# ZrrSkywalker/MonoDETR

Measured on NVIDIA H100. Metric: images/sec (1280x384, fwd+bwd), higher is better.
Workload: dtype f32 (BF16x3: error-compensated bf16 tensor-core products, fp32 accumulate)

## Files before the change

monodetr_b200/csrc/attention.cu:

```cuda
#include <cuda_runtime.h>
#include <math.h>
#include <stdint.h>

#include "../../include/monodetr_b200.h"
#include "launch.cuh"
#include "rng.cuh"
#include "tc_common.cuh"

namespace {

using namespace mdb;

constexpr int HD = 32;
constexpr int BR = 64;
constexpr int BC = 64;
constexpr int kTileBytes = BC * HD * 4;
constexpr int ATT_THREADS = 128;

struct AttnParams {
    const float *q, *k, *v;
    const uint8_t* kpm;
    float* out;
    float* lse;
    int B, H, Lq, Lk, ldq, ldk, ldv, ldo;
    float scale;
    float drop_p;
    const unsigned long long* seed;
    unsigned long long site;
    const float *dout, *o;
    float* delta;
    float *dq, *dk, *dv;
    int lddq, lddk, lddv;
};

__device__ __forceinline__ uint32_t f2tf32(float x) {
    uint32_t r;
    asm("cvt.rna.tf32.f32 %0, %1;" : "=r"(r) : "f"(x));
    return r;
}
__device__ __forceinline__ void split_tf32(float x, uint32_t& hi, uint32_t& lo) {
    hi = f2tf32(x);
    lo = f2tf32(x - __uint_as_float(hi));
}
struct AFrag {
    uint32_t hi[4][4];
    uint32_t lo[4][4];
};
__device__ __forceinline__ void load_afrag(AFrag& f, const float* base, int ld, int r0, int nrows, int lane, float mul) {
    const int g = lane >> 2, t = lane & 3;
    const int ra = r0 + g, rb = r0 + g + 8;
    const float* pa = base + (size_t)min(ra, nrows - 1) * ld;
    const float* pb = base + (size_t)min(rb, nrows - 1) * ld;
    const float ma = ra < nrows ? mul : 0.f, mb = rb < nrows ? mul : 0.f;
#pragma unroll
    for (int ks = 0; ks < 4; ++ks) {
        split_tf32(pa[ks * 8 + t] * ma, f.hi[ks][0], f.lo[ks][0]);
        split_tf32(pb[ks * 8 + t] * mb, f.hi[ks][1], f.lo[ks][1]);
        split_tf32(pa[ks * 8 + t + 4] * ma, f.hi[ks][2], f.lo[ks][2]);
        split_tf32(pb[ks * 8 + t + 4] * mb, f.hi[ks][3], f.lo[ks][3]);
    }
}

__device__ __forceinline__ uint32_t nt_off(int r, int c) { return (uint32_t)(r * 128 + ((((c >> 2) ^ (r & 7))) << 4) + (c & 3) * 4); }
__device__ __forceinline__ uint32_t nn_off(int r, int c) {
    const int kk = r & 31, q = kk & 7;
    const int kpos = (kk & ~7) + ((q & 1) ? 4 + (q >> 1) : (q >> 1));
    return (uint32_t)((r >> 5) * 4096 + c * 128 + ((((kpos >> 2) ^ (c & 7))) << 4) + (kpos & 3) * 4);
}

template <int NS>
__device__ __forceinline__ void gemm_nt(float (&c)[8][4], const AFrag& a, uint32_t th, uint32_t tl) {
    float (&d)[32] = reinterpret_cast<float (&)[32]>(c);
#pragma unroll
    for (int i = 0; i < 32; ++i) d[i] = 0.f;
    wgmma_fence();
#pragma unroll
    for (int ks = 0; ks < 4; ++ks) {
        const uint64_t bh = make_wgmma_desc_sw128(th + ks * 32);
        if (NS == 3) {
            const uint64_t bl = make_wgmma_desc_sw128(tl + ks * 32);
            wgmma_tf32_n64(d, a.lo[ks], bh, 1);
            wgmma_tf32_n64(d, a.hi[ks], bl, 1);
        }
        wgmma_tf32_n64(d, a.hi[ks], bh, 1);
    }
    wgmma_commit();
    wgmma_wait_all();
    wgmma_fence_operands(d);
}

template <int NS>
__device__ __forceinline__ void gemm_nn(float (&acc)[4][4], const float (&p)[8][4], uint32_t th, uint32_t tl) {
    float (&d)[16] = reinterpret_cast<float (&)[16]>(acc);
#pragma unroll
    for (int half = 0; half < 2; ++half) {
        uint32_t ah[4][4], al[4][4];
#pragma unroll
        for (int u = 0; u < 4; ++u) {
            const int kt = half * 4 + u;
            split_tf32(p[kt][0], ah[u][0], al[u][0]);
            split_tf32(p[kt][2], ah[u][1], al[u][1]);
            split_tf32(p[kt][1], ah[u][2], al[u][2]);
            split_tf32(p[kt][3], ah[u][3], al[u][3]);
        }
        wgmma_fence();
#pragma unroll
        for (int u = 0; u < 4; ++u) {
            const uint32_t off = half * 4096 + u * 32;
            const uint64_t bh = make_wgmma_desc_sw128(th + off);
            if (NS == 3) {
                const uint64_t bl = make_wgmma_desc_sw128(tl + off);
                wgmma_tf32_n32(d, al[u], bh, 1);
                wgmma_tf32_n32(d, ah[u], bl, 1);
            }
            wgmma_tf32_n32(d, ah[u], bh, 1);
        }
        wgmma_commit();
        wgmma_wait_all();
        wgmma_fence_operands(d);
    }
}

constexpr int STG = BC * HD;
__device__ __forceinline__ void stage_tile(float* stg, const float* base, int ld, int r0, int nrows) {
#pragma unroll
    for (int u = 0; u < 4; ++u) {
        const int i = threadIdx.x + u * ATT_THREADS;
        const int r = i >> 3, c = (i & 7) * 4;
        const bool ok = r0 + r < nrows;
        const float* src = ok ? base + ((size_t)(r0 + r) * ld + c) : base;
        const uint32_t dst = (uint32_t)__cvta_generic_to_shared(stg) + (uint32_t)i * 16u;
        const int nbytes = ok ? 16 : 0;
        asm volatile("cp.async.cg.shared.global [%0], [%1], 16, %2;" ::"r"(dst), "l"(src), "r"(nbytes) : "memory");
    }
}
__device__ __forceinline__ void stage_commit() { asm volatile("cp.async.commit_group;" ::: "memory"); }
__device__ __forceinline__ void stage_wait() { asm volatile("cp.async.wait_all;" ::: "memory"); }
__device__ __forceinline__ void unstage_tile(uint8_t* nt_hi, uint8_t* nt_lo, uint8_t* nn_hi, uint8_t* nn_lo, const float* stg) {
#pragma unroll
    for (int u = 0; u < 4; ++u) {
        const int i = threadIdx.x + u * ATT_THREADS;
        const int r = i >> 3, c = (i & 7) * 4;
        const float4 v = *reinterpret_cast<const float4*>(stg + i * 4);
        uint32_t h[4], l[4];
        split_tf32(v.x, h[0], l[0]); split_tf32(v.y, h[1], l[1]); split_tf32(v.z, h[2], l[2]); split_tf32(v.w, h[3], l[3]);
        if (nt_hi) *reinterpret_cast<uint4*>(nt_hi + nt_off(r, c)) = make_uint4(h[0], h[1], h[2], h[3]);
        if (nt_lo) *reinterpret_cast<uint4*>(nt_lo + nt_off(r, c)) = make_uint4(l[0], l[1], l[2], l[3]);
#pragma unroll
        for (int e = 0; e < 4; ++e) {
            if (nn_hi) *reinterpret_cast<uint32_t*>(nn_hi + nn_off(r, c + e)) = h[e];
            if (nn_lo) *reinterpret_cast<uint32_t*>(nn_lo + nn_off(r, c + e)) = l[e];
        }
    }
}
static_assert(BC * (HD / 4) == 4 * ATT_THREADS, "tile loader mapping");

__device__ __forceinline__ float quad_max(float v) {
    v = fmaxf(v, __shfl_xor_sync(0xffffffffu, v, 1));
    return fmaxf(v, __shfl_xor_sync(0xffffffffu, v, 2));
}
__device__ __forceinline__ float quad_sum(float v) {
    v += __shfl_xor_sync(0xffffffffu, v, 1);
    return v + __shfl_xor_sync(0xffffffffu, v, 2);
}

struct DropCtx {
    uint32_t key, thr;
    float inv_keep;
    bool on;
};
__device__ __forceinline__ DropCtx make_drop(const AttnParams& p, int b, int h) {
    DropCtx d;
    d.on = p.drop_p > 0.f;
    d.inv_keep = 1.f / (1.f - p.drop_p);
    d.thr = mdb::rng_thr16(p.drop_p);
    d.key = 0u;
    if (d.on) d.key = mdb::rng_key32(*p.seed + p.site * 0x9E3779B97F4A7C15ull, (unsigned long long)(b * p.H + h));
    return d;
}
__device__ __forceinline__ float keep_scale(const DropCtx& d, uint32_t row_base, int j) {
    return mdb::rng_keep16(d.key, row_base + (uint32_t)j, d.thr) ? d.inv_keep : 0.f;
}

__device__ __forceinline__ uint32_t fetch_dead(const AttnParams& p, int b, int k0) {
    const int j = k0 + (int)threadIdx.x;
    if (threadIdx.x >= BC) return 0u;
    if (j >= p.Lk) return 1u;
    return (p.kpm && p.kpm[(size_t)b * p.Lk + j]) ? 1u : 0u;
}

__global__ void __launch_bounds__(ATT_THREADS, 3)
attn_fwd_kernel(const AttnParams p) {
    extern __shared__ __align__(1024) uint8_t dyn_smem[];
    uint8_t* sKh = dyn_smem;
    uint8_t* sKl = sKh + kTileBytes;
    uint8_t* sVh = sKl + kTileBytes;
    uint8_t* sVl = sVh + kTileBytes;
    float* gK = reinterpret_cast<float*>(sVl + kTileBytes);
    float* gV = gK + STG;
    uint8_t* sDead = reinterpret_cast<uint8_t*>(gV + STG);
    const int b = blockIdx.z, h = blockIdx.y;
    const int warp = threadIdx.x >> 5, lane = threadIdx.x & 31;
    const int g = lane >> 2, t = lane & 3;
    const int r0 = blockIdx.x * BR + warp * 16;
    const float* qb = p.q + (size_t)b * p.Lq * p.ldq + h * HD;
    const float* kb = p.k + (size_t)b * p.Lk * p.ldk + h * HD;
    const float* vb = p.v + (size_t)b * p.Lk * p.ldv + h * HD;
    const DropCtx drop = make_drop(p, b, h);
    stage_tile(gK, kb, p.ldk, 0, p.Lk);
    stage_tile(gV, vb, p.ldv, 0, p.Lk);
    stage_commit();
    uint32_t ndead = fetch_dead(p, b, 0);
    AFrag qa;
    load_afrag(qa, qb, p.ldq, r0, p.Lq, lane, p.scale);
    float acc[4][4];
#pragma unroll
    for (int i = 0; i < 4; ++i) acc[i][0] = acc[i][1] = acc[i][2] = acc[i][3] = 0.f;
    float m0 = -INFINITY, m1 = -INFINITY, l0 = 0.f, l1 = 0.f;
    const int qi0 = r0 + g, qi1 = r0 + g + 8;
    const uint32_t rb0 = (uint32_t)qi0 * (uint32_t)p.Lk, rb1 = (uint32_t)qi1 * (uint32_t)p.Lk;

    for (int k0 = 0; k0 < p.Lk; k0 += BC) {
        stage_wait();
        __syncthreads();
        unstage_tile(sKh, sKl, nullptr, nullptr, gK);
        unstage_tile(nullptr, nullptr, sVh, sVl, gV);
        if (threadIdx.x < BC) sDead[threadIdx.x] = (uint8_t)ndead;
        mdb::fence_proxy_async_smem();
        __syncthreads();
        if (k0 + BC < p.Lk) {
            stage_tile(gK, kb, p.ldk, k0 + BC, p.Lk);
            stage_tile(gV, vb, p.ldv, k0 + BC, p.Lk);
            stage_commit();
            ndead = fetch_dead(p, b, k0 + BC);
        }
        float s[8][4];
        gemm_nt<3>(s, qa, mdb::smem_u32(sKh), mdb::smem_u32(sKl));
        float mx0 = -INFINITY, mx1 = -INFINITY;
#pragma unroll
        for (int nt = 0; nt < 8; ++nt) {
            const uchar2 dd = *reinterpret_cast<const uchar2*>(&sDead[nt * 8 + 2 * t]);
            if (dd.x) { s[nt][0] = -INFINITY; s[nt][2] = -INFINITY; }
            if (dd.y) { s[nt][1] = -INFINITY; s[nt][3] = -INFINITY; }
            mx0 = fmaxf(mx0, fmaxf(s[nt][0], s[nt][1]));
            mx1 = fmaxf(mx1, fmaxf(s[nt][2], s[nt][3]));
        }
        const float mn0 = fmaxf(m0, quad_max(mx0)), mn1 = fmaxf(m1, quad_max(mx1));
        const float c0 = (mn0 == -INFINITY) ? 1.f : __expf(m0 - mn0), c1 = (mn1 == -INFINITY) ? 1.f : __expf(m1 - mn1);
        l0 *= c0; l1 *= c1;
#pragma unroll
        for (int dn = 0; dn < 4; ++dn) { acc[dn][0] *= c0; acc[dn][1] *= c0; acc[dn][2] *= c1; acc[dn][3] *= c1; }
#pragma unroll
        for (int nt = 0; nt < 8; ++nt) {
#pragma unroll
            for (int e = 0; e < 2; ++e) {
                const int j = k0 + nt * 8 + 2 * t + e;
                float p0 = (mn0 == -INFINITY) ? 0.f : __expf(s[nt][e] - mn0);
                float p1 = (mn1 == -INFINITY) ? 0.f : __expf(s[nt][2 + e] - mn1);
                l0 += p0; l1 += p1;
                if (drop.on) {
                    p0 *= keep_scale(drop, rb0, j);
                    p1 *= keep_scale(drop, rb1, j);
                }
                s[nt][e] = p0; s[nt][2 + e] = p1;
            }
        }
        m0 = mn0; m1 = mn1;
        gemm_nn<3>(acc, s, mdb::smem_u32(sVh), mdb::smem_u32(sVl));
    }
    l0 = quad_sum(l0); l1 = quad_sum(l1);
    const float i0 = l0 > 0.f ? 1.f / l0 : 0.f, i1 = l1 > 0.f ? 1.f / l1 : 0.f;
    float* ob = p.out + (size_t)b * p.Lq * p.ldo + h * HD;
#pragma unroll
    for (int dn = 0; dn < 4; ++dn) {
        if (qi0 < p.Lq) *reinterpret_cast<float2*>(ob + (size_t)qi0 * p.ldo + dn * 8 + 2 * t) = make_float2(acc[dn][0] * i0, acc[dn][1] * i0);
        if (qi1 < p.Lq) *reinterpret_cast<float2*>(ob + (size_t)qi1 * p.ldo + dn * 8 + 2 * t) = make_float2(acc[dn][2] * i1, acc[dn][3] * i1);
    }
    if (t == 0) {
        float* lp = p.lse + ((size_t)b * p.H + h) * p.Lq;
        if (qi0 < p.Lq) lp[qi0] = l0 > 0.f ? m0 + __logf(l0) : -INFINITY;
        if (qi1 < p.Lq) lp[qi1] = l1 > 0.f ? m1 + __logf(l1) : -INFINITY;
    }
}

__global__ void attn_delta_kernel(const AttnParams p) {
    const long long idx = blockIdx.x * (long long)blockDim.x + threadIdx.x;
    const long long n = (long long)p.B * p.Lq * p.H;
    if (idx >= n) return;
    const int h = (int)(idx % p.H);
    const long long bi = idx / p.H;
    const int i = (int)(bi % p.Lq);
    const int b = (int)(bi / p.Lq);
    const float* a = p.dout + (size_t)bi * p.ldo + h * HD;
    const float* o = p.o + (size_t)bi * p.ldo + h * HD;
    float s = 0.f;
#pragma unroll
    for (int d = 0; d < HD; d += 4) {
        const float4 x = *reinterpret_cast<const float4*>(a + d);
        const float4 y = *reinterpret_cast<const float4*>(o + d);
        s += x.x * y.x + x.y * y.y + x.z * y.z + x.w * y.w;
    }
    p.delta[((size_t)b * p.H + h) * p.Lq + i] = s;
}

__global__ void __launch_bounds__(ATT_THREADS, 3)
attn_bwd_dq_kernel(const AttnParams p) {
    extern __shared__ __align__(1024) uint8_t dyn_smem[];
    uint8_t* sKh = dyn_smem;
    uint8_t* sKl = sKh + kTileBytes;
    uint8_t* sKn = sKl + kTileBytes;
    uint8_t* sVh = sKn + kTileBytes;
    float* gK = reinterpret_cast<float*>(sVh + kTileBytes);
    float* gV = gK + STG;
    uint8_t* sDead = reinterpret_cast<uint8_t*>(gV + STG);
    const int b = blockIdx.z, h = blockIdx.y;
    const int warp = threadIdx.x >> 5, lane = threadIdx.x & 31;
    const int g = lane >> 2, t = lane & 3;
    const int r0 = blockIdx.x * BR + warp * 16;
    const float* qb = p.q + (size_t)b * p.Lq * p.ldq + h * HD;
    const float* gb = p.dout + (size_t)b * p.Lq * p.ldo + h * HD;
    const float* kb = p.k + (size_t)b * p.Lk * p.ldk + h * HD;
    const float* vb = p.v + (size_t)b * p.Lk * p.ldv + h * HD;
    const DropCtx drop = make_drop(p, b, h);
    stage_tile(gK, kb, p.ldk, 0, p.Lk);
    stage_tile(gV, vb, p.ldv, 0, p.Lk);
    stage_commit();
    uint32_t ndead = fetch_dead(p, b, 0);
    AFrag qa, ga;
    load_afrag(qa, qb, p.ldq, r0, p.Lq, lane, p.scale);
    load_afrag(ga, gb, p.ldo, r0, p.Lq, lane, 1.f);
    const int qi0 = r0 + g, qi1 = r0 + g + 8;
    const uint32_t rb0 = (uint32_t)qi0 * (uint32_t)p.Lk, rb1 = (uint32_t)qi1 * (uint32_t)p.Lk;
    const size_t st = ((size_t)b * p.H + h) * p.Lq;
    float lse0 = qi0 < p.Lq ? p.lse[st + qi0] : INFINITY, lse1 = qi1 < p.Lq ? p.lse[st + qi1] : INFINITY;
    if (lse0 == -INFINITY) lse0 = INFINITY;
    if (lse1 == -INFINITY) lse1 = INFINITY;
    const float dl0 = qi0 < p.Lq ? p.delta[st + qi0] : 0.f, dl1 = qi1 < p.Lq ? p.delta[st + qi1] : 0.f;
    float acc[4][4];
#pragma unroll
    for (int i = 0; i < 4; ++i) acc[i][0] = acc[i][1] = acc[i][2] = acc[i][3] = 0.f;

    for (int k0 = 0; k0 < p.Lk; k0 += BC) {
        stage_wait();
        __syncthreads();
        unstage_tile(sKh, sKl, sKn, nullptr, gK);
        unstage_tile(sVh, nullptr, nullptr, nullptr, gV);
        if (threadIdx.x < BC) sDead[threadIdx.x] = (uint8_t)ndead;
        mdb::fence_proxy_async_smem();
        __syncthreads();
        if (k0 + BC < p.Lk) {
            stage_tile(gK, kb, p.ldk, k0 + BC, p.Lk);
            stage_tile(gV, vb, p.ldv, k0 + BC, p.Lk);
            stage_commit();
            ndead = fetch_dead(p, b, k0 + BC);
        }
        float s[8][4], dp[8][4];
        gemm_nt<3>(s, qa, mdb::smem_u32(sKh), mdb::smem_u32(sKl));
        gemm_nt<1>(dp, ga, mdb::smem_u32(sVh), 0u);
#pragma unroll
        for (int nt = 0; nt < 8; ++nt) {
            const uchar2 dd = *reinterpret_cast<const uchar2*>(&sDead[nt * 8 + 2 * t]);
#pragma unroll
            for (int e = 0; e < 2; ++e) {
                const int j = k0 + nt * 8 + 2 * t + e;
                const bool dead = e ? dd.y : dd.x;
                float p0 = dead ? 0.f : __expf(s[nt][e] - lse0);
                float p1 = dead ? 0.f : __expf(s[nt][2 + e] - lse1);
                float d0 = dp[nt][e], d1 = dp[nt][2 + e];
                if (drop.on) {
                    d0 *= keep_scale(drop, rb0, j);
                    d1 *= keep_scale(drop, rb1, j);
                }
                s[nt][e] = p0 * (d0 - dl0);
                s[nt][2 + e] = p1 * (d1 - dl1);
            }
        }
        gemm_nn<1>(acc, s, mdb::smem_u32(sKn), 0u);
    }
    float* ob = p.dq + (size_t)b * p.Lq * p.lddq + h * HD;
#pragma unroll
    for (int dn = 0; dn < 4; ++dn) {
        if (qi0 < p.Lq) *reinterpret_cast<float2*>(ob + (size_t)qi0 * p.lddq + dn * 8 + 2 * t) = make_float2(acc[dn][0] * p.scale, acc[dn][1] * p.scale);
        if (qi1 < p.Lq) *reinterpret_cast<float2*>(ob + (size_t)qi1 * p.lddq + dn * 8 + 2 * t) = make_float2(acc[dn][2] * p.scale, acc[dn][3] * p.scale);
    }
}

__global__ void __launch_bounds__(ATT_THREADS, 2)
attn_bwd_dkv_kernel(const AttnParams p) {
    extern __shared__ __align__(1024) uint8_t dyn_smem[];
    uint8_t* sQh = dyn_smem;
    uint8_t* sQl = sQh + kTileBytes;
    uint8_t* sQn = sQl + kTileBytes;
    uint8_t* sGh = sQn + kTileBytes;
    uint8_t* sGn = sGh + kTileBytes;
    float* gQ = reinterpret_cast<float*>(sGn + kTileBytes);
    float* gG = gQ + STG;
    float* sL = gG + STG;
    float* sD = sL + BC;
    const int b = blockIdx.z, h = blockIdx.y;
    const int warp = threadIdx.x >> 5, lane = threadIdx.x & 31;
    const int g = lane >> 2, t = lane & 3;
    const int r0 = blockIdx.x * BR + warp * 16;
    const float* qb = p.q + (size_t)b * p.Lq * p.ldq + h * HD;
    const float* gb = p.dout + (size_t)b * p.Lq * p.ldo + h * HD;
    const float* kb = p.k + (size_t)b * p.Lk * p.ldk + h * HD;
    const float* vb = p.v + (size_t)b * p.Lk * p.ldv + h * HD;
    const DropCtx drop = make_drop(p, b, h);
    const size_t st = ((size_t)b * p.H + h) * p.Lq;
    auto fetch_stats = [&](int q0, float& l, float& d) {
        const int i = q0 + (int)threadIdx.x;
        l = INFINITY; d = 0.f;
        if (threadIdx.x < BC && i < p.Lq) {
            l = p.lse[st + i];
            d = p.delta[st + i];
            if (l == -INFINITY) l = INFINITY;
        }
    };
    float nl, nd;
    stage_tile(gQ, qb, p.ldq, 0, p.Lq);
    stage_tile(gG, gb, p.ldo, 0, p.Lq);
    stage_commit();
    fetch_stats(0, nl, nd);
    AFrag ka, va;
    load_afrag(ka, kb, p.ldk, r0, p.Lk, lane, p.scale);
    load_afrag(va, vb, p.ldv, r0, p.Lk, lane, 1.f);
    const int kj0 = r0 + g, kj1 = r0 + g + 8;
    const bool dead0 = kj0 >= p.Lk || (p.kpm && p.kpm[(size_t)b * p.Lk + min(kj0, p.Lk - 1)]);
    const bool dead1 = kj1 >= p.Lk || (p.kpm && p.kpm[(size_t)b * p.Lk + min(kj1, p.Lk - 1)]);
    float dk[4][4], dv[4][4];
#pragma unroll
    for (int i = 0; i < 4; ++i) {
        dk[i][0] = dk[i][1] = dk[i][2] = dk[i][3] = 0.f;
        dv[i][0] = dv[i][1] = dv[i][2] = dv[i][3] = 0.f;
    }

    for (int q0 = 0; q0 < p.Lq; q0 += BC) {
        stage_wait();
        __syncthreads();
        unstage_tile(sQh, sQl, sQn, nullptr, gQ);
        unstage_tile(sGh, nullptr, sGn, nullptr, gG);
        if (threadIdx.x < BC) { sL[threadIdx.x] = nl; sD[threadIdx.x] = nd; }
        mdb::fence_proxy_async_smem();
        __syncthreads();
        if (q0 + BC < p.Lq) {
            stage_tile(gQ, qb, p.ldq, q0 + BC, p.Lq);
            stage_tile(gG, gb, p.ldo, q0 + BC, p.Lq);
            stage_commit();
            fetch_stats(q0 + BC, nl, nd);
        }
        float s[8][4], dp[8][4];
        gemm_nt<3>(s, ka, mdb::smem_u32(sQh), mdb::smem_u32(sQl));
        gemm_nt<1>(dp, va, mdb::smem_u32(sGh), 0u);
        float pd[8][4];
#pragma unroll
        for (int nt = 0; nt < 8; ++nt) {
            const float2 l2 = *reinterpret_cast<const float2*>(&sL[nt * 8 + 2 * t]);
            const float2 d2 = *reinterpret_cast<const float2*>(&sD[nt * 8 + 2 * t]);
#pragma unroll
            for (int e = 0; e < 2; ++e) {
                const int i = q0 + nt * 8 + 2 * t + e;
                const float lse = e ? l2.y : l2.x, dl = e ? d2.y : d2.x;
                float p0 = dead0 ? 0.f : __expf(s[nt][e] - lse);
                float p1 = dead1 ? 0.f : __expf(s[nt][2 + e] - lse);
                float d0 = dp[nt][e], d1 = dp[nt][2 + e];
                float w0 = p0, w1 = p1;
                if (drop.on) {
                    const uint32_t rb = (uint32_t)i * (uint32_t)p.Lk;
                    const float k0s = keep_scale(drop, rb, kj0), k1s = keep_scale(drop, rb, kj1);
                    w0 *= k0s; w1 *= k1s; d0 *= k0s; d1 *= k1s;
                }
                pd[nt][e] = w0; pd[nt][2 + e] = w1;
                s[nt][e] = p0 * (d0 - dl);
                s[nt][2 + e] = p1 * (d1 - dl);
            }
        }
        gemm_nn<1>(dv, pd, mdb::smem_u32(sGn), 0u);
        gemm_nn<1>(dk, s, mdb::smem_u32(sQn), 0u);
    }
    float* dkb = p.dk + (size_t)b * p.Lk * p.lddk + h * HD;
    float* dvb = p.dv + (size_t)b * p.Lk * p.lddv + h * HD;
#pragma unroll
    for (int dn = 0; dn < 4; ++dn) {
        if (kj0 < p.Lk) {
            *reinterpret_cast<float2*>(dkb + (size_t)kj0 * p.lddk + dn * 8 + 2 * t) = make_float2(dk[dn][0] * p.scale, dk[dn][1] * p.scale);
            *reinterpret_cast<float2*>(dvb + (size_t)kj0 * p.lddv + dn * 8 + 2 * t) = make_float2(dv[dn][0], dv[dn][1]);
        }
        if (kj1 < p.Lk) {
            *reinterpret_cast<float2*>(dkb + (size_t)kj1 * p.lddk + dn * 8 + 2 * t) = make_float2(dk[dn][2] * p.scale, dk[dn][3] * p.scale);
            *reinterpret_cast<float2*>(dvb + (size_t)kj1 * p.lddv + dn * 8 + 2 * t) = make_float2(dv[dn][2], dv[dn][3]);
        }
    }
}

constexpr int kFwdSmem = 4 * kTileBytes + 2 * STG * 4 + BC;
constexpr int kDqSmem = 4 * kTileBytes + 2 * STG * 4 + BC;
constexpr int kDkvSmem = 5 * kTileBytes + 2 * STG * 4 + 2 * BC * 4;

int check(const AttnParams& p) {
    if (p.B <= 0 || p.H <= 0 || p.Lq <= 0 || p.Lk <= 0) return MDB_EINVAL;
    if ((p.ldq | p.ldk | p.ldv | p.ldo) % 4) return MDB_EINVAL;
    if (p.drop_p < 0.f || p.drop_p >= 1.f) return MDB_EINVAL;
    if (p.drop_p > 0.f && !p.seed) return MDB_EINVAL;
    if (p.H > 65535 || p.B > 65535) return MDB_EUNSUPPORTED;
    if ((unsigned long long)p.Lq * (unsigned long long)p.Lk >= (1ull << 32)) return MDB_EUNSUPPORTED;
    return 0;
}

}

extern "C" {

int mdb_attention_forward_f32(const float* q, const float* k, const float* v, const unsigned char* key_padding_mask,
                              float* out, float* lse, int B, int H, int Lq, int Lk, int head_dim, int ldq, int ldk,
                              int ldv, int ldo, float drop_p, const unsigned long long* seed, unsigned long long site,
                              void* stream) {
    if (head_dim != HD) return MDB_EUNSUPPORTED;
    if (!q || !k || !v || !out || !lse) return MDB_EINVAL;
    AttnParams p{};
    p.q = q; p.k = k; p.v = v; p.kpm = key_padding_mask; p.out = out; p.lse = lse;
    p.B = B; p.H = H; p.Lq = Lq; p.Lk = Lk; p.ldq = ldq; p.ldk = ldk; p.ldv = ldv; p.ldo = ldo;
    p.scale = 1.f / sqrtf((float)HD); p.drop_p = drop_p; p.seed = seed; p.site = site;
    int rc = check(p);
    if (rc) return rc;
    dim3 grid((Lq + BR - 1) / BR, H, B);
    const cudaError_t e = set_max_dynamic_smem(attn_fwd_kernel, kFwdSmem);
    if (e != cudaSuccess) return (int)e;
    attn_fwd_kernel<<<grid, ATT_THREADS, kFwdSmem, static_cast<cudaStream_t>(stream)>>>(p);
    return (int)cudaGetLastError();
}

int mdb_attention_backward_f32(const float* q, const float* k, const float* v, const unsigned char* key_padding_mask,
                               const float* out, const float* lse, const float* dout, float* delta_ws, float* dq,
                               float* dk, float* dv, int B, int H, int Lq, int Lk, int head_dim, int ldq, int ldk, int ldv,
                               int ldo, int lddq, int lddk, int lddv, float drop_p, const unsigned long long* seed,
                               unsigned long long site, void* stream_) {
    if (head_dim != HD) return MDB_EUNSUPPORTED;
    if (!q || !k || !v || !out || !lse || !dout || !delta_ws || !dq || !dk || !dv) return MDB_EINVAL;
    cudaStream_t stream = static_cast<cudaStream_t>(stream_);
    AttnParams p{};
    p.q = q; p.k = k; p.v = v; p.kpm = key_padding_mask; p.lse = const_cast<float*>(lse);
    p.B = B; p.H = H; p.Lq = Lq; p.Lk = Lk; p.ldq = ldq; p.ldk = ldk; p.ldv = ldv; p.ldo = ldo;
    p.scale = 1.f / sqrtf((float)HD); p.drop_p = drop_p; p.seed = seed; p.site = site;
    p.dout = dout; p.o = out; p.delta = delta_ws; p.dq = dq; p.dk = dk; p.dv = dv;
    p.lddq = lddq; p.lddk = lddk; p.lddv = lddv;
    int rc = check(p);
    if (rc) return rc;
    if ((lddq | lddk | lddv) % 4) return MDB_EINVAL;
    const long long n = (long long)B * Lq * H;
    attn_delta_kernel<<<(unsigned)((n + 255) / 256), 256, 0, stream>>>(p);
    cudaError_t e = set_max_dynamic_smem(attn_bwd_dq_kernel, kDqSmem);
    if (e == cudaSuccess) e = set_max_dynamic_smem(attn_bwd_dkv_kernel, kDkvSmem);
    if (e != cudaSuccess) return (int)e;
    attn_bwd_dq_kernel<<<dim3((Lq + BR - 1) / BR, H, B), ATT_THREADS, kDqSmem, stream>>>(p);
    attn_bwd_dkv_kernel<<<dim3((Lk + BR - 1) / BR, H, B), ATT_THREADS, kDkvSmem, stream>>>(p);
    return (int)cudaGetLastError();
}

}
```

Baseline: 145.5.

## Overlap wgmma with dropout mask, vectorize nn unstaging, spill dK/dV fragments to smem

Splits gemm_nt into issue and wait so the QK^T and dP wgmmas run concurrently and the dropout keep-bits are computed while they are in flight. Separates tile unstaging into NT and NN variants, and the NN variant writes 16-byte vectors instead of scalar stores. In the dK/dV backward kernel the V-hi and K-lo A fragments are parked in shared memory and the result buffers are reused, which frees registers so launch bounds can be raised from 2 to 3 blocks per SM. The cost is extra shared memory per block and an smem reload of the fragments on every iteration.

```diff
diff --git a/monodetr_b200/csrc/attention.cu b/monodetr_b200/csrc/attention.cu
--- a/monodetr_b200/csrc/attention.cu
+++ b/monodetr_b200/csrc/attention.cu
@@ -69,7 +69,7 @@
 }
 
 template <int NS>
-__device__ __forceinline__ void gemm_nt(float (&c)[8][4], const AFrag& a, uint32_t th, uint32_t tl) {
+__device__ __forceinline__ void gemm_nt_issue(float (&c)[8][4], const AFrag& a, uint32_t th, uint32_t tl) {
     float (&d)[32] = reinterpret_cast<float (&)[32]>(c);
 #pragma unroll
     for (int i = 0; i < 32; ++i) d[i] = 0.f;
@@ -85,8 +85,15 @@
         wgmma_tf32_n64(d, a.hi[ks], bh, 1);
     }
     wgmma_commit();
+}
+__device__ __forceinline__ void gemm_nt_wait(float (&c0)[8][4], float (&c1)[8][4]) {
     wgmma_wait_all();
-    wgmma_fence_operands(d);
+    wgmma_fence_operands(reinterpret_cast<float (&)[32]>(c0));
+    wgmma_fence_operands(reinterpret_cast<float (&)[32]>(c1));
+}
+__device__ __forceinline__ void gemm_nt_wait(float (&c)[8][4]) {
+    wgmma_wait_all();
+    wgmma_fence_operands(reinterpret_cast<float (&)[32]>(c));
 }
 
 template <int NS>
@@ -136,7 +143,7 @@
 }
 __device__ __forceinline__ void stage_commit() { asm volatile("cp.async.commit_group;" ::: "memory"); }
 __device__ __forceinline__ void stage_wait() { asm volatile("cp.async.wait_all;" ::: "memory"); }
-__device__ __forceinline__ void unstage_tile(uint8_t* nt_hi, uint8_t* nt_lo, uint8_t* nn_hi, uint8_t* nn_lo, const float* stg) {
+__device__ __forceinline__ void unstage_nt(uint8_t* hi, uint8_t* lo, const float* stg) {
 #pragma unroll
     for (int u = 0; u < 4; ++u) {
         const int i = threadIdx.x + u * ATT_THREADS;
@@ -144,13 +151,21 @@
         const float4 v = *reinterpret_cast<const float4*>(stg + i * 4);
         uint32_t h[4], l[4];
         split_tf32(v.x, h[0], l[0]); split_tf32(v.y, h[1], l[1]); split_tf32(v.z, h[2], l[2]); split_tf32(v.w, h[3], l[3]);
-        if (nt_hi) *reinterpret_cast<uint4*>(nt_hi + nt_off(r, c)) = make_uint4(h[0], h[1], h[2], h[3]);
-        if (nt_lo) *reinterpret_cast<uint4*>(nt_lo + nt_off(r, c)) = make_uint4(l[0], l[1], l[2], l[3]);
-#pragma unroll
-        for (int e = 0; e < 4; ++e) {
-            if (nn_hi) *reinterpret_cast<uint32_t*>(nn_hi + nn_off(r, c + e)) = h[e];
-            if (nn_lo) *reinterpret_cast<uint32_t*>(nn_lo + nn_off(r, c + e)) = l[e];
-        }
+        *reinterpret_cast<uint4*>(hi + nt_off(r, c)) = make_uint4(h[0], h[1], h[2], h[3]);
+        if (lo) *reinterpret_cast<uint4*>(lo + nt_off(r, c)) = make_uint4(l[0], l[1], l[2], l[3]);
+    }
+}
+__device__ __forceinline__ void unstage_nn(uint8_t* hi, uint8_t* lo, const float* stg) {
+#pragma unroll
+    for (int u = 0; u < 4; ++u) {
+        const int i = threadIdx.x + u * ATT_THREADS;
+        const int c = i & 31, k = i >> 5;
+        const int r = (k >> 1) * 8 + (k & 1);
+        uint32_t h[4], l[4];
+#pragma unroll
+        for (int m = 0; m < 4; ++m) split_tf32(stg[(r + 2 * m) * HD + c], h[m], l[m]);
+        *reinterpret_cast<uint4*>(hi + nn_off(r, c)) = make_uint4(h[0], h[1], h[2], h[3]);
+        if (lo) *reinterpret_cast<uint4*>(lo + nn_off(r, c)) = make_uint4(l[0], l[1], l[2], l[3]);
     }
 }
 static_assert(BC * (HD / 4) == 4 * ATT_THREADS, "tile loader mapping");
@@ -178,8 +193,17 @@
     if (d.on) d.key = mdb::rng_key32(*p.seed + p.site * 0x9E3779B97F4A7C15ull, (unsigned long long)(b * p.H + h));
     return d;
 }
-__device__ __forceinline__ float keep_scale(const DropCtx& d, uint32_t row_base, int j) {
-    return mdb::rng_keep16(d.key, row_base + (uint32_t)j, d.thr) ? d.inv_keep : 0.f;
+__device__ __forceinline__ uint32_t keep_bits(const DropCtx& d, uint32_t row_base, int j0) {
+    uint32_t m = 0u;
+#pragma unroll
+    for (int nt = 0; nt < 8; ++nt)
+#pragma unroll
+        for (int e = 0; e < 2; ++e)
+            m |= (uint32_t)mdb::rng_keep16(d.key, row_base + (uint32_t)(j0 + nt * 8 + e), d.thr) << (2 * nt + e);
+    return m;
+}
+__device__ __forceinline__ float keep_scale(const DropCtx& d, uint32_t bits, int nt, int e) {
+    return (bits >> (2 * nt + e)) & 1u ? d.inv_keep : 0.f;
 }
 
 __device__ __forceinline__ uint32_t fetch_dead(const AttnParams& p, int b, int k0) {
@@ -223,8 +247,8 @@
     for (int k0 = 0; k0 < p.Lk; k0 += BC) {
         stage_wait();
         __syncthreads();
-        unstage_tile(sKh, sKl, nullptr, nullptr, gK);
-        unstage_tile(nullptr, nullptr, sVh, sVl, gV);
+        unstage_nt(sKh, sKl, gK);
+        unstage_nn(sVh, sVl, gV);
         if (threadIdx.x < BC) sDead[threadIdx.x] = (uint8_t)ndead;
         mdb::fence_proxy_async_smem();
         __syncthreads();
@@ -235,7 +259,10 @@
             ndead = fetch_dead(p, b, k0 + BC);
         }
         float s[8][4];
-        gemm_nt<3>(s, qa, mdb::smem_u32(sKh), mdb::smem_u32(sKl));
+        gemm_nt_issue<3>(s, qa, mdb::smem_u32(sKh), mdb::smem_u32(sKl));
+        uint32_t keep0 = 0u, keep1 = 0u;
+        if (drop.on) { keep0 = keep_bits(drop, rb0, k0 + 2 * t); keep1 = keep_bits(drop, rb1, k0 + 2 * t); }
+        gemm_nt_wait(s);
         float mx0 = -INFINITY, mx1 = -INFINITY;
 #pragma unroll
         for (int nt = 0; nt < 8; ++nt) {
@@ -254,13 +281,12 @@
         for (int nt = 0; nt < 8; ++nt) {
 #pragma unroll
             for (int e = 0; e < 2; ++e) {
-                const int j = k0 + nt * 8 + 2 * t + e;
                 float p0 = (mn0 == -INFINITY) ? 0.f : __expf(s[nt][e] - mn0);
                 float p1 = (mn1 == -INFINITY) ? 0.f : __expf(s[nt][2 + e] - mn1);
                 l0 += p0; l1 += p1;
                 if (drop.on) {
-                    p0 *= keep_scale(drop, rb0, j);
-                    p1 *= keep_scale(drop, rb1, j);
+                    p0 *= keep_scale(drop, keep0, nt, e);
+                    p1 *= keep_scale(drop, keep1, nt, e);
                 }
                 s[nt][e] = p0; s[nt][2 + e] = p1;
             }
@@ -343,8 +369,9 @@
     for (int k0 = 0; k0 < p.Lk; k0 += BC) {
         stage_wait();
         __syncthreads();
-        unstage_tile(sKh, sKl, sKn, nullptr, gK);
-        unstage_tile(sVh, nullptr, nullptr, nullptr, gV);
+        unstage_nt(sKh, sKl, gK);
+        unstage_nn(sKn, nullptr, gK);
+        unstage_nt(sVh, nullptr, gV);
         if (threadIdx.x < BC) sDead[threadIdx.x] = (uint8_t)ndead;
         mdb::fence_proxy_async_smem();
         __syncthreads();
@@ -355,21 +382,23 @@
             ndead = fetch_dead(p, b, k0 + BC);
         }
         float s[8][4], dp[8][4];
-        gemm_nt<3>(s, qa, mdb::smem_u32(sKh), mdb::smem_u32(sKl));
-        gemm_nt<1>(dp, ga, mdb::smem_u32(sVh), 0u);
+        gemm_nt_issue<3>(s, qa, mdb::smem_u32(sKh), mdb::smem_u32(sKl));
+        gemm_nt_issue<1>(dp, ga, mdb::smem_u32(sVh), 0u);
+        uint32_t keep0 = 0u, keep1 = 0u;
+        if (drop.on) { keep0 = keep_bits(drop, rb0, k0 + 2 * t); keep1 = keep_bits(drop, rb1, k0 + 2 * t); }
+        gemm_nt_wait(s, dp);
 #pragma unroll
         for (int nt = 0; nt < 8; ++nt) {
             const uchar2 dd = *reinterpret_cast<const uchar2*>(&sDead[nt * 8 + 2 * t]);
 #pragma unroll
             for (int e = 0; e < 2; ++e) {
-                const int j = k0 + nt * 8 + 2 * t + e;
                 const bool dead = e ? dd.y : dd.x;
                 float p0 = dead ? 0.f : __expf(s[nt][e] - lse0);
                 float p1 = dead ? 0.f : __expf(s[nt][2 + e] - lse1);
                 float d0 = dp[nt][e], d1 = dp[nt][2 + e];
                 if (drop.on) {
-                    d0 *= keep_scale(drop, rb0, j);
-                    d1 *= keep_scale(drop, rb1, j);
+                    d0 *= keep_scale(drop, keep0, nt, e);
+                    d1 *= keep_scale(drop, keep1, nt, e);
                 }
                 s[nt][e] = p0 * (d0 - dl0);
                 s[nt][2 + e] = p1 * (d1 - dl1);
@@ -385,7 +414,7 @@
     }
 }
 
-__global__ void __launch_bounds__(ATT_THREADS, 2)
+__global__ void __launch_bounds__(ATT_THREADS, 3)
 attn_bwd_dkv_kernel(const AttnParams p) {
     extern __shared__ __align__(1024) uint8_t dyn_smem[];
     uint8_t* sQh = dyn_smem;
@@ -397,6 +426,7 @@
     float* gG = gQ + STG;
     float* sL = gG + STG;
     float* sD = sL + BC;
+    uint4* sA = reinterpret_cast<uint4*>(sD + BC);
     const int b = blockIdx.z, h = blockIdx.y;
     const int warp = threadIdx.x >> 5, lane = threadIdx.x & 31;
     const int g = lane >> 2, t = lane & 3;
@@ -421,9 +451,18 @@
     stage_tile(gG, gb, p.ldo, 0, p.Lq);
     stage_commit();
     fetch_stats(0, nl, nd);
-    AFrag ka, va;
-    load_afrag(ka, kb, p.ldk, r0, p.Lk, lane, p.scale);
-    load_afrag(va, vb, p.ldv, r0, p.Lk, lane, 1.f);
+    uint32_t kah[4][4];
+    {
+        AFrag ka, va;
+        load_afrag(ka, kb, p.ldk, r0, p.Lk, lane, p.scale);
+        load_afrag(va, vb, p.ldv, r0, p.Lk, lane, 1.f);
+#pragma unroll
+        for (int ks = 0; ks < 4; ++ks) {
+            kah[ks][0] = ka.hi[ks][0]; kah[ks][1] = ka.hi[ks][1]; kah[ks][2] = ka.hi[ks][2]; kah[ks][3] = ka.hi[ks][3];
+            sA[ks * ATT_THREADS + threadIdx.x] = make_uint4(va.hi[ks][0], va.hi[ks][1], va.hi[ks][2], va.hi[ks][3]);
+            sA[(4 + ks) * ATT_THREADS + threadIdx.x] = make_uint4(ka.lo[ks][0], ka.lo[ks][1], ka.lo[ks][2], ka.lo[ks][3]);
+        }
+    }
     const int kj0 = r0 + g, kj1 = r0 + g + 8;
     const bool dead0 = kj0 >= p.Lk || (p.kpm && p.kpm[(size_t)b * p.Lk + min(kj0, p.Lk - 1)]);
     const bool dead1 = kj1 >= p.Lk || (p.kpm && p.kpm[(size_t)b * p.Lk + min(kj1, p.Lk - 1)]);
@@ -437,8 +476,10 @@
     for (int q0 = 0; q0 < p.Lq; q0 += BC) {
         stage_wait();
         __syncthreads();
-        unstage_tile(sQh, sQl, sQn, nullptr, gQ);
-        unstage_tile(sGh, nullptr, sGn, nullptr, gG);
+        unstage_nt(sQh, sQl, gQ);
+        unstage_nn(sQn, nullptr, gQ);
+        unstage_nt(sGh, nullptr, gG);
+        unstage_nn(sGn, nullptr, gG);
         if (threadIdx.x < BC) { sL[threadIdx.x] = nl; sD[threadIdx.x] = nd; }
         mdb::fence_proxy_async_smem();
         __syncthreads();
@@ -448,10 +489,20 @@
             stage_commit();
             fetch_stats(q0 + BC, nl, nd);
         }
+        AFrag ka, va;
+#pragma unroll
+        for (int ks = 0; ks < 4; ++ks) {
+            const uint4 v4 = sA[ks * ATT_THREADS + threadIdx.x], l4 = sA[(4 + ks) * ATT_THREADS + threadIdx.x];
+            va.hi[ks][0] = v4.x; va.hi[ks][1] = v4.y; va.hi[ks][2] = v4.z; va.hi[ks][3] = v4.w;
+            ka.lo[ks][0] = l4.x; ka.lo[ks][1] = l4.y; ka.lo[ks][2] = l4.z; ka.lo[ks][3] = l4.w;
+            ka.hi[ks][0] = kah[ks][0]; ka.hi[ks][1] = kah[ks][1]; ka.hi[ks][2] = kah[ks][2]; ka.hi[ks][3] = kah[ks][3];
+        }
         float s[8][4], dp[8][4];
-        gemm_nt<3>(s, ka, mdb::smem_u32(sQh), mdb::smem_u32(sQl));
-        gemm_nt<1>(dp, va, mdb::smem_u32(sGh), 0u);
-        float pd[8][4];
+        gemm_nt_issue<3>(s, ka, mdb::smem_u32(sQh), mdb::smem_u32(sQl));
+        gemm_nt_issue<1>(dp, va, mdb::smem_u32(sGh), 0u);
+        gemm_nt_wait(s, dp);
+        wgmma_fence_operands(ka.lo);
+        wgmma_fence_operands(va.hi);
 #pragma unroll
         for (int nt = 0; nt < 8; ++nt) {
             const float2 l2 = *reinterpret_cast<const float2*>(&sL[nt * 8 + 2 * t]);
@@ -466,16 +517,17 @@
                 float w0 = p0, w1 = p1;
                 if (drop.on) {
                     const uint32_t rb = (uint32_t)i * (uint32_t)p.Lk;
-                    const float k0s = keep_scale(drop, rb, kj0), k1s = keep_scale(drop, rb, kj1);
+                    const float k0s = mdb::rng_keep16(drop.key, rb + (uint32_t)kj0, drop.thr) ? drop.inv_keep : 0.f;
+                    const float k1s = mdb::rng_keep16(drop.key, rb + (uint32_t)kj1, drop.thr) ? drop.inv_keep : 0.f;
                     w0 *= k0s; w1 *= k1s; d0 *= k0s; d1 *= k1s;
                 }
-                pd[nt][e] = w0; pd[nt][2 + e] = w1;
-                s[nt][e] = p0 * (d0 - dl);
-                s[nt][2 + e] = p1 * (d1 - dl);
+                s[nt][e] = w0; s[nt][2 + e] = w1;
+                dp[nt][e] = p0 * (d0 - dl);
+                dp[nt][2 + e] = p1 * (d1 - dl);
             }
         }
-        gemm_nn<1>(dv, pd, mdb::smem_u32(sGn), 0u);
-        gemm_nn<1>(dk, s, mdb::smem_u32(sQn), 0u);
+        gemm_nn<1>(dv, s, mdb::smem_u32(sGn), 0u);
+        gemm_nn<1>(dk, dp, mdb::smem_u32(sQn), 0u);
     }
     float* dkb = p.dk + (size_t)b * p.Lk * p.lddk + h * HD;
     float* dvb = p.dv + (size_t)b * p.Lk * p.lddv + h * HD;
@@ -494,7 +546,8 @@
 
 constexpr int kFwdSmem = 4 * kTileBytes + 2 * STG * 4 + BC;
 constexpr int kDqSmem = 4 * kTileBytes + 2 * STG * 4 + BC;
-constexpr int kDkvSmem = 5 * kTileBytes + 2 * STG * 4 + 2 * BC * 4;
+constexpr int kDkvAFrag = 8 * ATT_THREADS * 16;
+constexpr int kDkvSmem = 5 * kTileBytes + 2 * STG * 4 + 2 * BC * 4 + kDkvAFrag;
 
 int check(const AttnParams& p) {
     if (p.B <= 0 || p.H <= 0 || p.Lq <= 0 || p.Lk <= 0) return MDB_EINVAL;
```

Result: no change. 145.4, median of 6 (-0.0%).
